# remi-or/fa2_triton

Hardware: AMD Instinct MI355X
Metric: attention TFLOP/s (fwd & fwd+bwd) at S=4096 D=128 bf16; % of MFMA peak (higher is better)
Workload: dtype bf16; 1 GPU; B=8 Hq=32 Hkv=32 S=4096 D=128 bf16 causal fwd+bwd per GPU (BASELINE.json configs[2]; configs[3] = B=64 batch-sharded over 8 GPUs); config=cfg3, global_batch=8, per_gpu_batch=8, seq_len=4096, heads=32, heads_kv=32, head_dim=128, causal=True, fwd_only=False, bias=False

## Files before the change

### fa2_triton_amd/csrc/dkdv_hp_kernel.h

```cpp
#pragma once
#include "common.h"
#include "fa2_internal.h"
#include "hp_unit.h"

namespace fa2 {

struct DkdvHpArgs {
  uint32_t qb0, qb1, vb0, vb1, ta, tb, lb, qoff0, qoff1, ooff0, ooff1, lsoff;
  uint32_t qb0h, qb1h, tah, tbh;
  int lr;
  int ng, nmt, c0, c01, c012, mlast, lq, kd0;
  uint32_t qrb, orb, qwrap, owrap, lwrap, lc0;
  uint32_t qlo, qhi, olo, ohi, lselo, lsehi, dllo, dlhi, mlds, lbs, w0;
  float sc;
  uint32_t mlo, mhi, mrange, mstep, mwrap;
  uint32_t dscb;
};

}

#include "gen/dkdv_hp_body.h"

namespace fa2 {

template <bool BF16, bool CAUSAL, bool DROPOUT>
FA2_DEV void dkdv_hp_main(const u32x4 (&kf)[16], const DkdvHpArgs& a) {
  if constexpr (DROPOUT) {
    if constexpr (BF16 && CAUSAL) dkdv_hp_main_bf16_causal_drop(kf, a);
    else if constexpr (BF16) dkdv_hp_main_bf16_full_drop(kf, a);
    else if constexpr (CAUSAL) dkdv_hp_main_f16_causal_drop(kf, a);
    else dkdv_hp_main_f16_full_drop(kf, a);
  } else {
    if constexpr (BF16 && CAUSAL) dkdv_hp_main_bf16_causal(kf, a);
    else if constexpr (BF16) dkdv_hp_main_bf16_full(kf, a);
    else if constexpr (CAUSAL) dkdv_hp_main_f16_causal(kf, a);
    else dkdv_hp_main_f16_full(kf, a);
  }
}

static_assert(DkdvLds<false>::v0 == 16384 * DkdvLds<false>::nbuf && DkdvLds<true>::rows == DkdvLds<true>::v0 + 65536,
              "dK/dV LDS layout");
constexpr int kDkdvStage = 32768;

struct DkdvBlk {
  int b, hkv, split, h0, G, Lq, Lk, n0, diag, n_mt, m_last, total;
};

template <bool CAUSAL>
FA2_DEV DkdvBlk dkdv_blk(const fa2_bwd_args& p, int nsplit, int item, int rep) {
  constexpr int BNK = 256, BMQ = 32;
  const int nkb = hp_blocks(p.seqlen_k), per_grp = hp_items_per_group<CAUSAL>(nkb);
  const int grp = item / per_grp, jb = item - grp * per_grp;
  DkdvBlk k;
  const int bkv = grp / nsplit;
  k.split = grp - bkv * nsplit;
  k.b = bkv / p.heads_kv;
  k.hkv = bkv - k.b * p.heads_kv;
  k.G = p.heads_q / p.heads_kv / nsplit;
  k.h0 = (k.hkv * nsplit + k.split) * k.G;
  k.Lq = p.seqlen_q;
  k.Lk = p.seqlen_k;
  if (p.cu_seqlens) k.Lq = k.Lk = p.cu_seqlens[k.b + 1] - p.cu_seqlens[k.b];
  k.n0 = (rep == 0 ? jb : nkb - 1 - jb) * BNK;
  k.diag = k.Lk - k.Lq;
  int m_begin = 0;
  if (CAUSAL) m_begin = max(0, k.n0 - k.diag) & ~(BMQ - 1);
  k.n_mt = (k.n0 < k.Lk && m_begin < k.Lq) ? (k.Lq - m_begin + BMQ - 1) / BMQ : 0;
  k.m_last = m_begin + (k.n_mt - 1) * BMQ;
  k.total = k.n_mt * k.G;
  return k;
}

FA2_DEV int dkdv_tiles_from(const DkdvBlk& k, int t) {
  return k.m_last < t ? 0 : min(((k.m_last - t) >> 5) + 1, k.n_mt);
}

template <bool CAUSAL>
FA2_DEV void dkdv_sched_dims(const fa2_bwd_args& p, int nsplit, int& T, int& nkb, int& per_grp) {
  nkb = hp_blocks(p.seqlen_k);
  per_grp = hp_items_per_group<CAUSAL>(nkb);
  T = per_grp * p.batch * p.heads_kv * nsplit;
}

FA2_DEV int64_t dkdv_mask_bytes(const fa2_bwd_args& p) {
  return 128ll * p.batch * p.heads_q * ((p.seqlen_q + 31) >> 5) * ((p.seqlen_k + 31) >> 5);
}
FA2_DEV uint32_t dkdv_mask_range(const fa2_bwd_args& p, int64_t off) {
  const int64_t r = dkdv_mask_bytes(p) - off;
  return r <= 0 ? 0u : r >= 0xFFFFFFFFll ? 0xFFFFFFFFu : (uint32_t)r;
}
FA2_DEV int64_t dkdv_mask_base(const fa2_bwd_args& p, const DkdvBlk& k, int w) {
  const int nrb = (p.seqlen_q + 31) >> 5, ncw = (p.seqlen_k + 31) >> 5;
  const int rt_min = (k.m_last >> 5) - (k.n_mt - 1);
  const int kt0 = (k.n0 + 64 * w) >> 5;
  return 128ll * (((int64_t)(k.b * p.heads_q + k.h0) * nrb + rt_min) * ncw + kt0);
}

typedef const __attribute__((address_space(4))) fa2_bwd_args* dkdv_kargs_t;
FA2_DEV const fa2_bwd_args* dkdv_kargs() {
  dkdv_kargs_t pa = (dkdv_kargs_t)__builtin_amdgcn_kernarg_segment_ptr();
  asm volatile("" : "+s"(pa));
  return (const fa2_bwd_args*)pa;
}

FA2_DEV int dkdv_lane() {
  int lane;
  asm volatile("v_mbcnt_lo_u32_b32 %0, -1, 0\n\tv_mbcnt_hi_u32_b32 %0, -1, %0" : "=v"(lane));
  return lane;
}

template <bool CAUSAL, bool DROPOUT>
FA2_DEV uint32_t dkdv_hp_issue(const fa2_bwd_args& p, const DkdvBlk& k, char* smem, int w, int lane, u32x4 (&kf)[16],
                               bool live = true) {
  constexpr int DT = 128, BMQ = 32, NT = 256;
  const int tid = 64 * w + lane, r32 = lane & 31, hh = lane >> 5, D = p.head_dim;
  const int kw0 = k.n0 + 64 * w;
  const uint32_t sb = lds_addr(smem);
  uint32_t tok = 0;
  if (live && k.total > 0) {
    const uint16_t* vg = (const uint16_t*)p.v + k.b * p.v_stride[0] + k.hkv * p.v_stride[2];
    BufStager<DT, 64, 64> vst;
    vst.init(lane, p.v_stride[1], D);
    tok = vst.issue(smem + DkdvLds<DROPOUT>::v0 + 16384 * w, vg, p.v_stride[1], kw0, k.Lk, BufStager<DT, 64, 64>::max_rows(p.v_stride[1]));
    BufStager<DT, BMQ, NT> qst, ost;
    qst.init(tid, p.q_stride[1], D);
    ost.init(tid, p.do_stride[1], D);
    const uint16_t* q0 = (const uint16_t*)p.q + k.b * p.q_stride[0] + k.h0 * p.q_stride[2];
    const uint16_t* o0 = (const uint16_t*)p.dout + k.b * p.do_stride[0] + k.h0 * p.do_stride[2];
    tok += qst.issue(smem, q0, p.q_stride[1], k.m_last, k.Lq, BufStager<DT, BMQ, NT>::max_rows(p.q_stride[1]));
    tok += ost.issue(smem + 8192, o0, p.do_stride[1], k.m_last, k.Lq, BufStager<DT, BMQ, NT>::max_rows(p.do_stride[1]));
    const int64_t l0 = (int64_t)(k.b * p.heads_q + k.h0) * p.lse_row_stride + k.m_last;
    if (w == 0) {
      const uint32_t nb = (uint32_t)min(k.Lq - k.m_last, BMQ) * 4u;
      blds4_lo32(4u * (uint32_t)lane, make_rsrc(p.lse + l0, nb), __builtin_amdgcn_readfirstlane(sb + DkdvLds<DROPOUT>::rows));
      blds4_lo32(4u * (uint32_t)lane, make_rsrc(p.delta + l0, nb), __builtin_amdgcn_readfirstlane(sb + DkdvLds<DROPOUT>::rows + 128));
    }
    if constexpr (DROPOUT) {
      const int ncw = (p.seqlen_k + 31) >> 5;
      const int64_t moff = dkdv_mask_base(p, k, w) + 128ll * ncw * (k.n_mt - 1);
      const char* mw = (const char*)p.dropout_mask + moff;
      blds4(4u * (uint32_t)lane, make_rsrc(mw, min(dkdv_mask_range(p, moff), 256u)), __builtin_amdgcn_readfirstlane(sb + DkdvLds<DROPOUT>::words + 256 * w));
    }
  }
#pragma unroll
  for (int kb = 0; kb < 2; ++kb) {
    const int kj = kw0 + 32 * kb + r32;
    const bool kval = kj < k.Lk;
    const uint16_t* krow = (const uint16_t*)p.k + k.b * p.k_stride[0] + k.hkv * p.k_stride[2] + (int64_t)(kval ? kj : 0) * p.k_stride[1];
#pragma unroll
    for (int ks = 0; ks < 8; ++ks) kf[kb * 8 + ks] = load_row_frag<true>(krow, 16 * ks + 8 * hh, D, kval);
  }
  return __builtin_amdgcn_readfirstlane(tok);
}

template <bool BF16, bool CAUSAL, bool DROPOUT>
__global__ void __launch_bounds__(256, 1) dkdv_hp_kernel(const fa2_bwd_args p_, int nsplit
#if FA2_HP_STAMPS
                                                         , unsigned long long* stamps
#endif
) {
  HpStamps st;
  constexpr int DT = 128, BMQ = 32, NT = 256;
  __shared__ __attribute__((aligned(16))) char smem[DkdvLds<DROPOUT>::size];

  const int w_ = __builtin_amdgcn_readfirstlane(threadIdx.x >> 6);
  int w = w_;
  PersistSched sch;
  {
    int T, nkb, per_grp;
    dkdv_sched_dims<CAUSAL>(p_, nsplit, T, nkb, per_grp);
    if (!sch.first(T, nkb, per_grp, CAUSAL)) return;
  }
  u32x4 kf[16];
  {
    const int lane = dkdv_lane();
    const auto& p = *dkdv_kargs();
    (void)dkdv_hp_issue<CAUSAL, DROPOUT>(p, dkdv_blk<CAUSAL>(p, nsplit, sch.item, sch.rep), smem, w, lane, kf);
  }

  st.start();
  while (true) {
    const int lane = dkdv_lane();
    w = w_;
    asm volatile("" : "+s"(w));
    const int tid = 64 * w + lane, r32 = lane & 31, hh = lane >> 5;
    {
      const auto& p = *dkdv_kargs();
      const DkdvBlk k = dkdv_blk<CAUSAL>(p, nsplit, sch.item, sch.rep);
      const int D = p.head_dim;
      const int kw0 = k.n0 + 64 * w;
      const float sc = p.softmax_scale * kLog2e;
      const uint32_t sb = lds_addr(smem);
      BufStager<DT, BMQ, NT> qst, ost;
      qst.init(tid, p.q_stride[1], D);
      ost.init(tid, p.do_stride[1], D);
      const int64_t q_rb = p.q_stride[1] * 2, o_rb = p.do_stride[1] * 2;
      const uint16_t* q0 = (const uint16_t*)p.q + k.b * p.q_stride[0] + k.h0 * p.q_stride[2];
      const uint16_t* o0 = (const uint16_t*)p.dout + k.b * p.do_stride[0] + k.h0 * p.do_stride[2];
      const int64_t l0 = (int64_t)(k.b * p.heads_q + k.h0) * p.lse_row_stride + k.m_last;

      DkdvHpArgs a;
      a.qb0 = hp_row_frag_base(sb, r32, hh, 0);
      a.qb1 = hp_row_frag_base(sb, r32, hh, 1);
      a.vb0 = a.qb0 + DkdvLds<DROPOUT>::v0 + 16384 * w;
      a.vb1 = a.qb1 + DkdvLds<DROPOUT>::v0 + 16384 * w;
      {
        const int i = lane & 15, g = lane >> 4, h = lane >> 5;
        const int qq = i >> 2, pq = i & 3;
        const int cc = 2 * (g & 1) + (pq >> 1);
        const int base = (4 * h + qq) * 64 + 8 * (pq & 1);
        a.ta = sb + base + ((cc ^ h) << 4);
        a.tb = sb + base + 512 + ((cc ^ h ^ 2) << 4);
      }
      a.qb0h = a.qb0 + 65536;
      a.qb1h = a.qb1 + 65536;
      a.tah = a.ta + 65536;
      a.tbh = a.tb + 65536;
      a.lb = sb + DkdvLds<DROPOUT>::rows + 16 * hh;
      a.qoff0 = qst.voff[0];
      a.qoff1 = qst.voff[1];
      a.ooff0 = ost.voff[0];
      a.ooff1 = ost.voff[1];
      a.lsoff = 4 * lane;
      a.lr = r32 - 4 * hh;
      a.kd0 = __builtin_amdgcn_readfirstlane(kw0 - k.diag);
      int c0, c1, c2;
      {
        const int live = kw0 >= k.Lk ? 0 : CAUSAL ? dkdv_tiles_from(k, kw0 - (BMQ - 1) - k.diag) : k.n_mt;
        const int clear = kw0 + 63 >= k.Lk ? 0 : CAUSAL ? dkdv_tiles_from(k, kw0 + 63 - k.diag) : k.n_mt;
        const int tail = k.m_last + BMQ > k.Lq ? 1 : 0;
        c1 = max(min(clear, live) - tail, 0);
        c0 = c1 > 0 ? tail : live;
        c2 = c1 > 0 ? live - clear : 0;
      }
      a.ng = __builtin_amdgcn_readfirstlane(k.G);
      a.nmt = __builtin_amdgcn_readfirstlane(k.n_mt);
      a.c0 = __builtin_amdgcn_readfirstlane(c0);
      a.c01 = __builtin_amdgcn_readfirstlane(c0 + c1);
      a.c012 = __builtin_amdgcn_readfirstlane(c0 + c1 + c2);
      a.mlast = __builtin_amdgcn_readfirstlane(k.m_last);
      a.lq = __builtin_amdgcn_readfirstlane(k.Lq);
      a.qrb = __builtin_amdgcn_readfirstlane((uint32_t)q_rb);
      a.orb = __builtin_amdgcn_readfirstlane((uint32_t)o_rb);
      a.qwrap = __builtin_amdgcn_readfirstlane((uint32_t)((int64_t)(k.n_mt - 1) * BMQ * q_rb + 2 * p.q_stride[2]));
      a.owrap = __builtin_amdgcn_readfirstlane((uint32_t)((int64_t)(k.n_mt - 1) * BMQ * o_rb + 2 * p.do_stride[2]));
      a.lwrap = __builtin_amdgcn_readfirstlane((uint32_t)(((int64_t)(k.n_mt - 1) * BMQ + p.lse_row_stride) * 4));
      a.lc0 = __builtin_amdgcn_readfirstlane((uint32_t)(l0 * 4));
      const uint64_t qa = (uint64_t)(uintptr_t)q0 + (uint64_t)((int64_t)k.m_last * q_rb);
      const uint64_t oa = (uint64_t)(uintptr_t)o0 + (uint64_t)((int64_t)k.m_last * o_rb);
      a.qlo = sgpr_lo(qa), a.qhi = sgpr_hi(qa);
      a.olo = sgpr_lo(oa), a.ohi = sgpr_hi(oa);
      const uint64_t la = (uint64_t)(uintptr_t)p.lse, da = (uint64_t)(uintptr_t)p.delta;
      a.lselo = sgpr_lo(la), a.lsehi = sgpr_hi(la);
      a.dllo = sgpr_lo(da), a.dlhi = sgpr_hi(da);
      a.mlds = __builtin_amdgcn_readfirstlane(sb + (uint32_t)w * 1024u);
      a.lbs = __builtin_amdgcn_readfirstlane(sb + (uint32_t)DkdvLds<DROPOUT>::rows);
      a.w0 = __builtin_amdgcn_readfirstlane((uint32_t)w);
      a.sc = sc;
      if constexpr (DROPOUT) {
        const uint32_t lds_part = sb + (uint32_t)DkdvLds<DROPOUT>::words + 256u * (uint32_t)w;
        a.lsoff = lds_part + 4 * lane;
        const int nrb = (p.seqlen_q + 31) >> 5, ncw = (p.seqlen_k + 31) >> 5;
        const uint64_t mb = ((uint64_t)(uintptr_t)p.dropout_mask + (uint64_t)dkdv_mask_base(p, k, w) - lds_part) & kAddr48;
        a.mlo = sgpr_lo(mb), a.mhi = sgpr_hi(mb);
        a.mrange = __builtin_amdgcn_readfirstlane(dkdv_mask_range(p, dkdv_mask_base(p, k, w) - (int64_t)lds_part));
        a.mstep = __builtin_amdgcn_readfirstlane((uint32_t)(128 * ncw));
        a.mwrap = __builtin_amdgcn_readfirstlane((uint32_t)(128 * ncw * (nrb + k.n_mt - 1)));
        a.dscb = __float_as_uint(1.f / (1.f - p.dropout_p));
        const uint64_t la2 = la - lds_part, da2 = da - lds_part;
        a.lselo = sgpr_lo(la2), a.lsehi = sgpr_hi(la2);
        a.dllo = sgpr_lo(da2), a.dlhi = sgpr_hi(da2);
      }

      st.mark(7);
      dkdv_hp_main<BF16, CAUSAL, DROPOUT>(kf, a);
      st.mark(0);
      st.count(5);
    }

    PersistSched nsch = sch;
    bool has_next;
    {
      const auto& p = *dkdv_kargs();
      int T, nkb, per_grp;
      dkdv_sched_dims<CAUSAL>(p, nsplit, T, nkb, per_grp);
      has_next = nsch.next(T, nkb, per_grp, CAUSAL);
    }
    uint32_t tok;
    {
      const auto& p = *dkdv_kargs();
      tok = dkdv_hp_issue<CAUSAL, DROPOUT>(p, dkdv_blk<CAUSAL>(p, nsplit, has_next ? nsch.item : sch.item, has_next ? nsch.rep : sch.rep), smem,
                                  w, lane, kf, has_next);
    }
    asm volatile("" ::: "memory");
    st.mark(1);

    {
      const auto& p = *dkdv_kargs();
      const DkdvBlk k = dkdv_blk<CAUSAL>(p, nsplit, sch.item, sch.rep);
      const int D = p.head_dim;
      const int kw0 = k.n0 + 64 * w;
      const float scale = p.softmax_scale;
      const float vscale = DROPOUT ? 1.f / (1.f - p.dropout_p) : 1.f;
#pragma unroll
      for (int kb = 0; kb < 2; ++kb) {
        f32x16 dv[4], dk[4];
        if (kb == 0) dkdv_hp_read<0>(dv, dk, tok);
        else dkdv_hp_read<1>(dv, dk, tok);
        st.mark(kb ? 4 : 2);
        const int kwb = kw0 + 32 * kb;
        const int kj = kwb + r32;
        const bool kval = kj < k.Lk;
        if (nsplit > 1) {
          if (kj < p.seqlen_k) {
            const int64_t row = (((int64_t)k.split * p.batch + k.b) * p.heads_kv + k.hkv) * p.seqlen_k + kj;
            float* pk = p.dkv_workspace + row * D;
            float* pv = p.dkv_workspace + ((int64_t)nsplit * p.batch * p.heads_kv * p.seqlen_k + row) * D;
#pragma unroll
            for (int dt = 0; dt < 4; ++dt)
#pragma unroll
              for (int g4 = 0; g4 < 4; ++g4) {
                const int d0 = 32 * dt + 8 * g4 + 4 * hh;
                f32x4 x, y;
#pragma unroll
                for (int j = 0; j < 4; ++j) {
                  x[j] = kval ? dk[dt][4 * g4 + j] : 0.f;
                  y[j] = kval ? dv[dt][4 * g4 + j] * vscale : 0.f;
                }
                *(f32x4*)(pk + d0) = x;
                *(f32x4*)(pv + d0) = y;
              }
          }
        } else if (kwb < p.seqlen_k) {
          uint16_t* k0 = (uint16_t*)p.dk + k.b * p.dk_stride[0] + k.hkv * p.dk_stride[2] + (int64_t)kwb * p.dk_stride[1];
          uint16_t* v0 = (uint16_t*)p.dv + k.b * p.dv_stride[0] + k.hkv * p.dv_stride[2] + (int64_t)kwb * p.dv_stride[1];
          const int nrows = min(32, p.seqlen_k - kwb);
          char* stage = smem + kDkdvStage + w * 32 * DT * 2;
          store_rows_lds<BF16, DT>(stage, dk, scale, kval, k0, p.dk_stride[1], nrows, D, lane, st.parts());
          store_rows_lds<BF16, DT>(stage, dv, vscale, kval, v0, p.dv_stride[1], nrows, D, lane, st.parts());
        }
        st.mark(kb ? 6 : 3);
      }
    }
    if (!has_next) break;
    sch = nsch;
  }
  asm volatile("s_waitcnt vmcnt(0)" ::: "memory");
#if FA2_HP_STAMPS
  st.flush(stamps, dkdv_lane());
#endif
}

template <bool BF16, bool CAUSAL, bool DROPOUT>
static void launch_dkdv_hp(const fa2_bwd_args& a, int nsplit, LaunchCtx ctx) {
  const int64_t items = hp_sched_items<CAUSAL>(a.seqlen_k, (int64_t)a.batch * a.heads_kv * nsplit);
  dim3 grid((unsigned)hp_grid(items, device_cu_count(), ctx.policy));
#if FA2_HP_STAMPS
  hipLaunchKernelGGL((dkdv_hp_kernel<BF16, CAUSAL, DROPOUT>), grid, dim3(256), 0, ctx.stream, a, nsplit, hp_stamp_buf());
#else
  hipLaunchKernelGGL((dkdv_hp_kernel<BF16, CAUSAL, DROPOUT>), grid, dim3(256), 0, ctx.stream, a, nsplit);
#endif
}

}
```

### fa2_triton_amd/csrc/dq_hp_kernel.h

```cpp
#pragma once
#include "common.h"
#include "fa2_internal.h"
#include "hp_unit.h"

namespace fa2 {

struct DqHpArgs {
  uint32_t kb0, kb1, ta, tb;
  uint32_t off0, off1, off2, off3;
  int rel0, rel1;
  float lse0, lse1, del0, del1;
  int na, last, ntiles;
  uint32_t tileb, kbytes, mlds, klo, khi, vlo, vhi;
  float sc;
  int boff;
  uint32_t nklo, nkhi, nvlo, nvhi, nkbytes, nqlo, nqhi, nqbytes, nolo, nohi, nobytes;
  uint32_t nqo0, noo0;
  uint32_t nqrs, nors;
  u32x4 mdesc;
  uint32_t mo0, nmo0, msh, mrs;
  float dsc;
};

}

#include "gen/dq_hp_body.h"

namespace fa2 {

template <bool BF16, bool CAUSAL, bool DROPOUT>
FA2_DEV void dq_hp_main(u32x4 (&q)[16], u32x4 (&o)[16], const DqHpArgs& a, uint32_t (&mw)[4]) {
  if constexpr (DROPOUT) {
    if constexpr (BF16 && CAUSAL) dq_hp_main_bf16_causal_drop(q, o, a, mw);
    else if constexpr (BF16) dq_hp_main_bf16_full_drop(q, o, a, mw);
    else if constexpr (CAUSAL) dq_hp_main_f16_causal_drop(q, o, a, mw);
    else dq_hp_main_f16_full_drop(q, o, a, mw);
  } else {
    if constexpr (BF16 && CAUSAL) dq_hp_main_bf16_causal(q, o, a);
    else if constexpr (BF16) dq_hp_main_bf16_full(q, o, a);
    else if constexpr (CAUSAL) dq_hp_main_f16_causal(q, o, a);
    else dq_hp_main_f16_full(q, o, a);
  }
}

template <bool CAUSAL>
struct DqHpUnit : HpRowUnit<CAUSAL> {
  const uint16_t *kg, *vg, *qg, *dg, *og;
  FA2_DEV void init(const fa2_bwd_args& p, HpWalk at) {
    const int hkv = HpRowUnit<CAUSAL>::init(p.heads_q, p.heads_kv, p.seqlen_q, p.seqlen_k, p.cu_seqlens, at.bh, at.mb);
    const int b = this->b, hq = this->hq;
    kg = (const uint16_t*)p.k + b * p.k_stride[0] + hkv * p.k_stride[2];
    vg = (const uint16_t*)p.v + b * p.v_stride[0] + hkv * p.v_stride[2];
    qg = (const uint16_t*)p.q + b * p.q_stride[0] + hq * p.q_stride[2];
    dg = (const uint16_t*)p.dout + b * p.do_stride[0] + hq * p.do_stride[2];
    og = (const uint16_t*)p.o + b * p.o_stride[0] + hq * p.o_stride[2];
  }
};

template <bool BF16, bool CAUSAL>
FA2_DEV void dq_hp_unit_rows(const fa2_bwd_args& p, const DqHpUnit<CAUSAL>& u, int qw0, int hh, int r32,
                             const u32x4 (&of)[16], float (&lse)[2], float (&del)[2]) {
  using E = Elem<BF16>;
  const int D = p.head_dim;
  const int64_t srow = (int64_t)(u.b * p.heads_q + u.hq) * p.lse_row_stride;
#pragma unroll
  for (int rb = 0; rb < 2; ++rb) {
    const int qi = qw0 + 32 * rb + r32;
    const bool qvalid = qi < u.Lq;
    const uint16_t* orow = u.og + (int64_t)(qvalid ? qi : 0) * p.o_stride[1];
    float part = 0.f;
#pragma unroll
    for (int ks = 0; ks < 8; ++ks) {
      const u32x4 orr = load_row_frag<true>(orow, 16 * ks + 8 * hh, D, qvalid);
      const u32x4 dr = of[rb * 8 + ks];
#pragma unroll
      for (int j = 0; j < 4; ++j) {
        part = fmaf(E::to_f32((uint16_t)(orr[j] & 0xFFFF)), E::to_f32((uint16_t)(dr[j] & 0xFFFF)), part);
        part = fmaf(E::to_f32((uint16_t)(orr[j] >> 16)), E::to_f32((uint16_t)(dr[j] >> 16)), part);
      }
    }
    del[rb] = qvalid ? half_sum(part) : 0.f;
    if (hh == 0 && qi < p.lse_row_stride) p.delta[srow + qi] = -del[rb];
    lse[rb] = qvalid ? p.lse[srow + qi] : 0.f;
  }
}

template <bool BF16, bool CAUSAL, bool DROPOUT>
__global__ void __launch_bounds__(256, 1) dq_hp_kernel(const fa2_bwd_args p
#if FA2_HP_STAMPS
                                                       , unsigned long long* stamps
#endif
) {
  HpStamps st;
  constexpr int DT = 128, BN = 64, NT = 256;
  constexpr int TILE = BN * DT * 2;
  __shared__ __attribute__((aligned(16))) char smem[4 * TILE + 4 * 32 * DT * 2];

  const int w = __builtin_amdgcn_readfirstlane(threadIdx.x >> 6);
  constexpr bool PAIR = CAUSAL;
  const int nmb = hp_blocks(p.seqlen_q), per_bh = hp_items_per_group<PAIR>(nmb);
  const int T = per_bh * p.batch * p.heads_q;
  PersistSched sch;
  if (!sch.first(T, nmb, per_bh, PAIR)) return;

  int tid = threadIdx.x;
  const int lane = tid & 63, r32 = lane & 31, hh = lane >> 5;
  const int D = p.head_dim;
  const float scale = p.softmax_scale, sc = scale * kLog2e;
  const uint32_t sb = lds_addr(smem);
  const uint32_t rowb = (uint32_t)(p.k_stride[1] * 2);
  const uint32_t qrowb = (uint32_t)(p.q_stride[1] * 2), orowb = (uint32_t)(p.do_stride[1] * 2);
  BufStager<DT, BN, NT> kst;
  kst.init(tid, p.k_stride[1], D);
  const int mrows = BufStager<DT, BN, NT>::max_rows(p.k_stride[1]);

  DqHpUnit<CAUSAL> u;
  u.init(p, hp_walk_unit(sch, nmb, per_bh, PAIR));
  u32x4 qf[16], of[16];
  float lse[2], del[2];
  {
    if (u.ntiles > 0) {
      kst.issue(smem, u.kg, p.k_stride[1], 0, u.Lk, mrows);
      kst.issue(smem + 2 * TILE, u.vg, p.v_stride[1], 0, u.Lk, mrows);
    }
    const int qw0 = u.m0 + 64 * w;
#pragma unroll
    for (int rb = 0; rb < 2; ++rb) {
      const int qi = qw0 + 32 * rb + r32;
      const bool qvalid = qi < u.Lq;
      const uint16_t* qrow = u.qg + (int64_t)(qvalid ? qi : 0) * p.q_stride[1];
      const uint16_t* drow = u.dg + (int64_t)(qvalid ? qi : 0) * p.do_stride[1];
#pragma unroll
      for (int ks = 0; ks < 8; ++ks) {
        qf[rb * 8 + ks] = load_row_frag<true>(qrow, 16 * ks + 8 * hh, D, qvalid);
        of[rb * 8 + ks] = load_row_frag<true>(drow, 16 * ks + 8 * hh, D, qvalid);
      }
    }
    dq_hp_unit_rows<BF16, CAUSAL>(p, u, qw0, hh, r32, of, lse, del);
  }
  int boff = 0;
  const int nrb = (p.seqlen_q + 31) >> 5, ncw = (p.seqlen_k + 31) >> 5;
  const uint32_t mbytes = DROPOUT ? (uint32_t)((int64_t)p.batch * p.heads_q * nrb * ncw * 128) : 0u;
  auto mask_off = [&](const DqHpUnit<CAUSAL>& x, int rb) -> uint32_t {
    const int rbi = (x.m0 + 64 * w + 32 * rb) >> 5;
    return (uint32_t)(((int64_t)(x.b * p.heads_q + x.hq) * nrb + rbi) * ncw * 128) + 4u * r32;
  };
  uint32_t mw[4] = {0u, 0u, 0u, 0u};
  if constexpr (DROPOUT) {
#pragma unroll
    for (int rb = 0; rb < 2; ++rb)
#pragma unroll
      for (int h = 0; h < 2; ++h) {
        const uint32_t off = mask_off(u, rb) + 128u * h;
        mw[2 * rb + h] = off < mbytes ? p.dropout_mask[off >> 2] : 0u;
      }
  }

  st.start();
  while (true) {
    asm volatile("" : "+v"(tid));
    const int qw0 = u.m0 + 64 * w;
    const int diag = u.Lk - u.Lq;
    PersistSched nsch = sch;
    const bool has_next = nsch.next(T, nmb, per_bh, PAIR);
    DqHpUnit<CAUSAL> nu;
    nu.init(p, hp_walk_unit(has_next ? nsch : sch, nmb, per_bh, PAIR));
    auto next_rows = [&](DqHpArgs& x) {
      const int nqw0 = nu.m0 + 64 * w;
      const int nrows = has_next ? min(max(nu.Lq - nqw0, 0), 64) : 0;
      const int64_t r0 = nrows > 0 ? nqw0 : 0;
      const uint16_t *nq = nu.qg + r0 * p.q_stride[1], *no = nu.dg + r0 * p.do_stride[1];
      x.nqlo = sgpr_lo(nq), x.nqhi = sgpr_hi(nq);
      x.nolo = sgpr_lo(no), x.nohi = sgpr_hi(no);
      x.nqbytes = __builtin_amdgcn_readfirstlane(row_range_bytes(nrows, qrowb));
      x.nobytes = __builtin_amdgcn_readfirstlane(row_range_bytes(nrows, orowb));
      x.nqo0 = (uint32_t)r32 * qrowb + 16u * hh;
      x.noo0 = (uint32_t)r32 * orowb + 16u * hh;
      x.nqrs = __builtin_amdgcn_readfirstlane(32u * qrowb);
      x.nors = __builtin_amdgcn_readfirstlane(32u * orowb);
    };

    DqHpArgs a;
    a.kb0 = hp_row_frag_base(sb, r32, hh, 0);
    a.kb1 = hp_row_frag_base(sb, r32, hh, 1);
    {
      const int i = lane & 15, g = lane >> 4, h = lane >> 5;
      const int qq = i >> 2, pq = i & 3;
      const int cc = 2 * (g & 1) + (pq >> 1);
      const int base = (4 * h + qq) * 64 + 8 * (pq & 1);
      a.ta = sb + base + ((cc ^ h) << 4);
      a.tb = sb + base + 512 + ((cc ^ h ^ 2) << 4);
    }
    a.off0 = kst.voff[0];
    a.off1 = kst.voff[1];
    a.off2 = kst.voff[2];
    a.off3 = kst.voff[3];
#pragma unroll
    for (int rb = 0; rb < 2; ++rb) {
      const int qi = qw0 + 32 * rb + r32;
      const int lim = qi >= u.Lq ? 0 : (CAUSAL ? min(u.Lk, qi + diag + 1) : u.Lk);
      (rb ? a.rel1 : a.rel0) = lim - 4 * hh;
    }
    a.lse0 = lse[0];
    a.lse1 = lse[1];
    a.del0 = del[0];
    a.del1 = del[1];
    const int ntiles = u.ntiles;
    int n_full = u.Lk / BN;
    if (CAUSAL) n_full = min(n_full, qw0 + diag + 1 >= 0 ? (qw0 + diag + 1) / BN : 0);
    const bool live0 = ntiles > 0 && !(CAUSAL && 0 > qw0 + 63 + diag);
    int last = -1;
    if (live0) {
      last = ntiles - 1;
      if (CAUSAL) last = min(last, (qw0 + 63 + diag) / BN);
    }
    a.na = __builtin_amdgcn_readfirstlane(min(n_full, last + 1));
    a.last = __builtin_amdgcn_readfirstlane(last);
    a.ntiles = __builtin_amdgcn_readfirstlane(ntiles);
    a.tileb = __builtin_amdgcn_readfirstlane(BN * rowb);
    a.kbytes = __builtin_amdgcn_readfirstlane(kv_range_bytes(u.Lk, mrows, rowb));
    a.mlds = __builtin_amdgcn_readfirstlane(sb + (uint32_t)w * 1024u);
    a.klo = sgpr_lo(u.kg), a.khi = sgpr_hi(u.kg);
    a.vlo = sgpr_lo(u.vg), a.vhi = sgpr_hi(u.vg);
    a.sc = sc;
    a.boff = __builtin_amdgcn_readfirstlane(boff);
    {
      a.nklo = sgpr_lo(nu.kg), a.nkhi = sgpr_hi(nu.kg);
      a.nvlo = sgpr_lo(nu.vg), a.nvhi = sgpr_hi(nu.vg);
      a.nkbytes = __builtin_amdgcn_readfirstlane(has_next && nu.ntiles > 0 ? kv_range_bytes(nu.Lk, mrows, rowb) : 0u);
      if constexpr (!DROPOUT) next_rows(a);
    }
    if constexpr (DROPOUT) {
      a.mo0 = mask_off(u, 0);
      a.nmo0 = has_next ? mask_off(nu, 0) : 0x7FFFFFF0u;
      a.mrs = __builtin_amdgcn_readfirstlane((uint32_t)ncw * 128u);
      a.msh = 4u * hh;
      const uint64_t ma = (uint64_t)(uintptr_t)p.dropout_mask & kAddr48;
      a.mdesc[0] = sgpr_lo(ma), a.mdesc[1] = sgpr_hi(ma);
      a.mdesc[2] = __builtin_amdgcn_readfirstlane(mbytes);
      a.mdesc[3] = 0x20000u;
      a.dsc = 1.f / (1.f - p.dropout_p);
    }

    st.mark(8);
    dq_hp_main<BF16, CAUSAL, DROPOUT>(qf, of, a, mw);
    st.mark(0);
    st.count(5);
    f32x16 acc[2][4];
    dq_hp_read(acc);
    st.mark(2);

    char* stage = smem + 4 * TILE + w * 32 * DT * 2;
#pragma unroll
    for (int rb = 0; rb < 2; ++rb) {
      const int r0 = qw0 + 32 * rb;
      if (r0 < p.seqlen_q) {
        const bool qvalid = r0 + r32 < u.Lq;
        uint16_t* q0 = (uint16_t*)p.dq + u.b * p.dq_stride[0] + u.hq * p.dq_stride[2] + (int64_t)r0 * p.dq_stride[1];
        store_rows_lds<BF16, DT>(stage, acc[rb], scale, qvalid, q0, p.dq_stride[1], min(32, p.seqlen_q - r0), D, lane, st.parts());
      }
      st.mark(3 + rb);
    }
    if (!has_next) break;
    if constexpr (DROPOUT) {
      DqHpArgs na;
      next_rows(na);
      dq_hp_load_next(qf, of, na);
      st.mark(12);
    }
    asm volatile("s_nop 14\n\ts_waitcnt vmcnt(0)"
                 : "+a"(qf[0]), "+a"(qf[1]), "+a"(qf[2]), "+a"(qf[3]), "+a"(qf[4]), "+a"(qf[5]), "+a"(qf[6]),
                   "+a"(qf[7]), "+a"(qf[8]), "+a"(qf[9]), "+a"(qf[10]), "+a"(qf[11]), "+a"(qf[12]), "+a"(qf[13]),
                   "+a"(qf[14]), "+a"(qf[15]), "+a"(of[0]), "+a"(of[1]), "+a"(of[2]), "+a"(of[3]), "+a"(of[4]),
                   "+a"(of[5]), "+a"(of[6]), "+a"(of[7]), "+a"(of[8]), "+a"(of[9]), "+a"(of[10]), "+a"(of[11]),
                   "+a"(of[12]), "+a"(of[13]), "+a"(of[14]), "+a"(of[15]), "+v"(mw[0]), "+v"(mw[1]), "+v"(mw[2]),
                   "+v"(mw[3])
                 :
                 : "memory");
    st.mark(6);
    dq_hp_unit_rows<BF16, CAUSAL>(p, nu, nu.m0 + 64 * w, hh, r32, of, lse, del);
    st.mark(7);
    boff = (boff + ntiles) & 1;
    sch = nsch;
    u = nu;
  }
  asm volatile("s_waitcnt vmcnt(0)" ::: "memory");
#if FA2_HP_STAMPS
  st.flush(stamps, lane);
#endif
}

template <bool BF16, bool CAUSAL, bool DROPOUT>
static void launch_dq_hp(const fa2_bwd_args& a, LaunchCtx ctx) {
  const int64_t items = hp_sched_items<CAUSAL>(a.seqlen_q, (int64_t)a.batch * a.heads_q);
  dim3 grid((unsigned)hp_grid(items, device_cu_count(), ctx.policy));
#if FA2_HP_STAMPS
  hipLaunchKernelGGL((dq_hp_kernel<BF16, CAUSAL, DROPOUT>), grid, dim3(256), 0, ctx.stream, a, hp_stamp_buf());
#else
  hipLaunchKernelGGL((dq_hp_kernel<BF16, CAUSAL, DROPOUT>), grid, dim3(256), 0, ctx.stream, a);
#endif
}

}
```

### fa2_triton_amd/csrc/hp_unit.h

```cpp
#pragma once
#include <stdint.h>

#ifdef __HIP__
#define FA2_HD __host__ __device__ __forceinline__
#else
#define FA2_HD inline
#endif

namespace fa2 {
constexpr int kHpBlock = 256;
constexpr int kHpTile = 64;

FA2_HD int hp_min(int a, int b) { return a < b ? a : b; }
FA2_HD int hp_max(int a, int b) { return a > b ? a : b; }

template <bool CAUSAL>
struct HpRowUnit {
  int b, hq, Lq, Lk, m0, ntiles;
  FA2_HD int init(int heads_q, int heads_kv, int seqlen_q, int seqlen_k, const int32_t* cu_seqlens, int bh, int mb) {
    b = bh / heads_q;
    hq = bh - b * heads_q;
    const int hkv = hq / (heads_q / heads_kv);
    Lq = seqlen_q;
    Lk = seqlen_k;
    if (cu_seqlens) {
      const int cu = cu_seqlens[b];
      Lq = Lk = cu_seqlens[b + 1] - cu;
    }
    m0 = mb * kHpBlock;
    int n_end = 0;
    if (m0 < Lq) {
      n_end = Lk;
      if (CAUSAL) n_end = hp_min(Lk, m0 + kHpBlock + Lk - Lq);
      n_end = hp_max(n_end, 0);
    }
    ntiles = (n_end + kHpTile - 1) / kHpTile;
    return hkv;
  }
};

template <bool CAUSAL>
FA2_HD int hp_n_full(int Lk, int diag, int qw0) {
  int n_full = Lk / kHpTile;
  if (CAUSAL) n_full = hp_min(n_full, qw0 + diag + 1 >= 0 ? (qw0 + diag + 1) / kHpTile : 0);
  return n_full;
}
template <bool CAUSAL>
FA2_HD int hp_last_tile(int diag, int qw0, int ntiles) {
  const bool live0 = ntiles > 0 && !(CAUSAL && 0 > qw0 + 63 + diag);
  int last = -1;
  if (live0) {
    last = ntiles - 1;
    if (CAUSAL) last = hp_min(last, (qw0 + 63 + diag) / kHpTile);
  }
  return last;
}

FA2_HD int hp_blocks(int seqlen) { return (seqlen + kHpBlock - 1) / kHpBlock; }
template <bool PAIR>
FA2_HD int hp_items_per_group(int n) { return PAIR ? (n + 1) / 2 : n; }
template <bool PAIR>
FA2_HD int64_t hp_sched_items(int seqlen, int64_t groups) { return hp_items_per_group<PAIR>(hp_blocks(seqlen)) * groups; }

FA2_HD uint32_t kv_range_bytes(int Lk, int mrows, uint32_t rowb) { return (uint32_t)hp_min(Lk, mrows) * rowb; }
FA2_HD uint32_t row_range_bytes(int nrows, uint32_t rowb) { return nrows > 0 ? (uint32_t)(nrows - 1) * rowb + 256u : 0u; }
}

#ifdef __HIP__
#include "common.h"
namespace fa2 {
struct HpWalk { int bh, mb; };
FA2_DEV HpWalk hp_walk_unit(const PersistSched& s, int nmb, int per_bh, bool pair) {
  HpWalk r;
  r.bh = s.item / per_bh;
  const int mbi = s.item - r.bh * per_bh;
  r.mb = pair && s.rep == 0 ? nmb - 1 - mbi : mbi;
  return r;
}

FA2_DEV uint32_t sgpr_lo(uint64_t a) { return __builtin_amdgcn_readfirstlane((uint32_t)a); }
FA2_DEV uint32_t sgpr_hi(uint64_t a) { return __builtin_amdgcn_readfirstlane((uint32_t)(a >> 32)); }
FA2_DEV uint32_t sgpr_lo(const void* p) { return sgpr_lo((uint64_t)(uintptr_t)p); }
FA2_DEV uint32_t sgpr_hi(const void* p) { return sgpr_hi((uint64_t)(uintptr_t)p); }
constexpr uint64_t kAddr48 = 0xFFFFFFFFFFFFull;
}
#endif
```

### fa2_triton_amd/csrc/select.h

```cpp
#pragma once
#include <stdint.h>

#include "fa2_amd.h"

namespace fa2 {

inline bool path_enabled(const fa2_policy* policy, uint32_t bit) { return !(policy && (policy->disable & bit)); }
inline int hp_grid(int64_t items, int ncu, const fa2_policy* policy) {
  const int cap = policy ? policy->grid_cap : 0;
  if (cap > 0 && cap < ncu) ncu = cap;
  return (int)(items < ncu ? items : ncu);
}

inline int head_dim_tile(int d) { return d <= 32 ? 32 : d <= 64 ? 64 : d <= 128 ? 128 : d <= 256 ? 256 : 0; }

inline bool bias16_rows(const void* bias, int dtype, const int64_t* stride) {
  return bias && (dtype == 16 || dtype == 17) && ((uintptr_t)bias & 15) == 0 && stride[0] % 8 == 0 &&
         stride[1] % 8 == 0 && stride[2] % 8 == 0;
}

inline bool fwd_hp_ok(const fa2_fwd_args& a, bool aligned, const fa2_policy* policy) {
  if (!path_enabled(policy, FA2_PATH_FWD_HP) || !aligned || a.head_dim != 128 || a.bias) return false;
#if FA2_HP_STAMPS
  if (a.dropout_p > 0.f) return false;
#endif
  if (a.dropout_p > 0.f &&
      (!a.dropout_mask || (int64_t)a.batch * a.heads_q * ((a.seqlen_q + 31) / 32) * ((a.seqlen_k + 31) / 32) * 128 >= ((int64_t)1 << 31)))
    return false;
  if (a.k_stride[1] != a.v_stride[1]) return false;
  return (int64_t)(a.seqlen_k + 128) * a.k_stride[1] * 2 < ((int64_t)1 << 31);
}

inline bool dq_hp_ok(const fa2_bwd_args& a, bool aligned, const fa2_policy* policy) {
  if (!path_enabled(policy, FA2_PATH_DQ_HP) || !aligned || a.head_dim != 128 || a.bias || a.dq_dtype != a.dtype) return false;
  if (a.dropout_p > 0.f) {
    if (!a.dropout_mask) return false;
    const int64_t nrb = (a.seqlen_q + 31) / 32, ncw = (a.seqlen_k + 31) / 32;
    if ((int64_t)a.batch * a.heads_q * nrb * ncw * 128 >= ((int64_t)1 << 31)) return false;
  }
  if (a.k_stride[1] != a.v_stride[1]) return false;
  const int64_t lim = (int64_t)1 << 31;
  return (int64_t)(a.seqlen_k + 128) * a.k_stride[1] * 2 < lim && (int64_t)64 * a.q_stride[1] * 2 < lim &&
         (int64_t)64 * a.do_stride[1] * 2 < lim;
}

inline bool dkdv_hp_ok(const fa2_bwd_args& a, bool aligned, const fa2_policy* policy) {
  if (!path_enabled(policy, FA2_PATH_DKDV_HP) || !aligned || a.head_dim != 128 || a.bias) return false;
  const int64_t lim = (int64_t)1 << 31;
  if (a.dropout_p > 0.f) {
    if (!a.dropout_mask || a.q_stride[1] != a.do_stride[1]) return false;
    const int64_t nrb = (a.seqlen_q + 31) / 32, ncw = (a.seqlen_k + 31) / 32;
    if ((int64_t)(a.heads_q / a.heads_kv) * nrb * ncw * 128 >= lim) return false;
  }
  const int64_t lse_bytes = (int64_t)a.batch * a.heads_q * a.lse_row_stride * 4;
  if (a.q_stride[2] < 0 || a.do_stride[2] < 0) return false;
  return (int64_t)(a.seqlen_q + 64) * a.q_stride[1] * 2 + 2 * a.q_stride[2] < lim &&
         (int64_t)(a.seqlen_q + 64) * a.do_stride[1] * 2 + 2 * a.do_stride[2] < lim && lse_bytes < lim;
}

constexpr int kDkvTargetGrid = 512;
inline int dkv_split_count(int B, int Hq, int Hkv, int Sk) {
  if (B < 1 || Hkv < 1 || Hq % Hkv != 0 || Sk < 1) return 1;
  const int G = Hq / Hkv;
  const int64_t grid = (int64_t)((Sk + 127) / 128) * B * Hkv;
  if (G <= 1 || grid >= kDkvTargetGrid) return 1;
  for (int s = 2; s < G; ++s)
    if (G % s == 0 && grid * s >= kDkvTargetGrid) return s;
  return G;
}
inline int64_t dkv_workspace_bytes(int B, int Hq, int Hkv, int Sk, int D) {
  const int s = dkv_split_count(B, Hq, Hkv, Sk);
  return s > 1 ? 2 * (int64_t)s * B * Hkv * Sk * D * 4 : 0;
}
inline int dkv_split(const fa2_bwd_args& a) {
  return a.dkv_workspace ? dkv_split_count(a.batch, a.heads_q, a.heads_kv, a.seqlen_k) : 1;
}

enum class Path : int { general, pipelined, hand_placed, local };

struct FwdPlan {
  Path path;
  bool causal, aligned, mask_first;
  int biask, drop;
};

inline FwdPlan select_fwd(const fa2_fwd_args& a, bool aligned, const fa2_policy* policy) {
  const bool bias = a.bias != nullptr, dropout = a.dropout_p > 0.f;
  if (a.local) return {Path::local, false, aligned, false, 0, 0};
  const int drop = dropout ? (a.dropout_mask ? 2 : 1) : 0, dt = head_dim_tile(a.head_dim);
  FwdPlan p = {Path::general, a.causal != 0, aligned, drop == 2, bias ? 1 : 0, drop};
  if (fwd_hp_ok(a, aligned, policy)) {
    p.path = Path::hand_placed;
  } else if ((dt == 64 || dt == 128) && aligned && !dropout && a.k_stride[1] == a.v_stride[1] &&
             (!bias || bias16_rows(a.bias, a.bias_dtype, a.bias_stride))) {
    p.path = Path::pipelined;
    p.biask = !bias ? 0 : (a.bias_dtype == FA2_BF16 ? 17 : 16);
  }
  return p;
}

enum class Stage : int { delta, dq, dbias, dkdv };
struct BwdPlan {
  bool causal, dropout, aligned, dq_f32;
  int biask;
  struct {
    Stage kind;
    Path path;
  } stage[4];
  int nstages;
  int nsplit;
  bool reduce;
};

inline BwdPlan select_bwd(const fa2_bwd_args& a, bool aligned, int stages, const fa2_policy* policy) {
  BwdPlan p = {};
  const bool bias = a.bias != nullptr;
  p.causal = !a.local && a.causal != 0;
  p.dropout = a.dropout_p > 0.f;
  p.aligned = aligned;
  p.dq_f32 = a.dq_dtype == FA2_F32;
  p.nsplit = 1;
  if (bias) p.biask = aligned && bias16_rows(a.bias, a.bias_dtype, a.bias_stride) ? (a.bias_dtype == FA2_BF16 ? 17 : 16) : 1;
  const Path local_or = a.local ? Path::local : Path::general;
  auto add = [&](Stage kind, Path path) {
    p.stage[p.nstages].kind = kind;
    p.stage[p.nstages++].path = path;
  };
  if ((stages & 1) && a.lse_row_stride > 0) add(Stage::delta, Path::general);
  if ((stages & 4) && a.seqlen_q > 0) add(Stage::dq, !a.local && dq_hp_ok(a, aligned, policy) ? Path::hand_placed : local_or);
  if ((stages & 8) && bias && a.dbias && a.seqlen_q > 0 && a.seqlen_k > 0) add(Stage::dbias, Path::general);
  if ((stages & 2) && a.seqlen_k > 0) {
    add(Stage::dkdv, !a.local && dkdv_hp_ok(a, aligned, policy) ? Path::hand_placed : local_or);
    if (!a.local) p.nsplit = dkv_split(a);
    p.reduce = p.nsplit > 1;
  }
  return p;
}

inline const fa2_kvcache_args& kv_base(const fa2_kvcache_args& a) { return a; }
inline const fa2_kvcache_args& kv_base(const fa2_paged_kvcache_args& a) { return a.base; }
inline const fa2_kvcache_args& kv_base(const fa2_fp8_kvcache_args& a) { return a.paged.base; }

inline int kv_row_tiles(const fa2_kvcache_args& a) {
  return (int)(((int64_t)(a.heads_q / a.heads_kv) * a.seqlen_q + 31) / 32);
}
inline int64_t kv_units(const fa2_kvcache_args& a) { return (int64_t)a.batch * a.heads_kv * kv_row_tiles(a); }

inline int kv_span_tiles(const fa2_kvcache_args& a) {
  int64_t span = a.capacity;
  if (a.window_left >= 0) {
    const int64_t band = (int64_t)a.window_left + a.seqlen_q + 63;
    if (band < span) span = band;
  }
  const int64_t t = (span + 63) / 64;
  return (int)(t < 1 ? 1 : t);
}

inline int kv_auto_splits(const fa2_kvcache_args& a, int ncu) {
  const int64_t units = kv_units(a);
  int64_t want = (2 * (int64_t)ncu + units - 1) / units;
  const int64_t most = kv_span_tiles(a) / FA2_KVCACHE_MIN_SPLIT_TILES;
  if (want > most) want = most;
  if (want > FA2_KVCACHE_MAX_SPLITS) want = FA2_KVCACHE_MAX_SPLITS;
  return (int)(want < 1 ? 1 : want);
}

inline int64_t kv_workspace_bytes(const fa2_kvcache_args& a, int nsplit) {
  if (nsplit <= 1) return 0;
  return (int64_t)nsplit * a.batch * a.heads_q * a.seqlen_q * ((int64_t)a.head_dim + 1) * 4;
}

constexpr int kFp8MaxHeadDim = 128;
inline int fp8_head_dim_tile(int d) { return d <= 64 ? 64 : d <= kFp8MaxHeadDim ? 128 : 0; }
inline bool fp8_paged(const fa2_fp8_kvcache_args& a) { return a.paged.block_table != nullptr; }
inline bool fp8_rows16(const void* cache, const int64_t* stride) {
  return ((uintptr_t)cache & 15) == 0 && stride[0] % 16 == 0 && stride[1] % 16 == 0 && stride[2] % 16 == 0;
}

}
```

Before: 940.2 TFLOP/s.

## Load K and O rows coalesced via buffer loads and transpose through LDS

In the dK/dV and dQ backward kernels, the per-lane strided row-fragment global loads for K (and for O in dQ's delta computation) are replaced. The new path issues coalesced 16-byte buffer loads across 4-row groups, then scatters them into a swizzled LDS image and reads them back in MFMA fragment layout. In dQ, the O request for the next unit is issued early so its latency overlaps the dQ store phase. This adds LDS traffic and register pressure for the raw staging arrays, and the hand-placed path now requires extra stride-eligibility checks.

Result: no change. 944.5 TFLOP/s, median of 6 (+0.5%).

```diff
diff --git a/fa2_triton_amd/csrc/dkdv_hp_kernel.h b/fa2_triton_amd/csrc/dkdv_hp_kernel.h
--- a/fa2_triton_amd/csrc/dkdv_hp_kernel.h
+++ b/fa2_triton_amd/csrc/dkdv_hp_kernel.h
@@ -110,10 +110,10 @@
 }
 
 template <bool CAUSAL, bool DROPOUT>
-FA2_DEV uint32_t dkdv_hp_issue(const fa2_bwd_args& p, const DkdvBlk& k, char* smem, int w, int lane, u32x4 (&kf)[16],
+FA2_DEV uint32_t dkdv_hp_issue(const fa2_bwd_args& p, const DkdvBlk& k, char* smem, int w, int lane, u32x4 (&kraw)[16],
                                bool live = true) {
   constexpr int DT = 128, BMQ = 32, NT = 256;
-  const int tid = 64 * w + lane, r32 = lane & 31, hh = lane >> 5, D = p.head_dim;
+  const int tid = 64 * w + lane, D = p.head_dim;
   const int kw0 = k.n0 + 64 * w;
   const uint32_t sb = lds_addr(smem);
   uint32_t tok = 0;
@@ -142,15 +142,16 @@
       blds4(4u * (uint32_t)lane, make_rsrc(mw, min(dkdv_mask_range(p, moff), 256u)), __builtin_amdgcn_readfirstlane(sb + DkdvLds<DROPOUT>::words + 256 * w));
     }
   }
-#pragma unroll
-  for (int kb = 0; kb < 2; ++kb) {
-    const int kj = kw0 + 32 * kb + r32;
-    const bool kval = kj < k.Lk;
-    const uint16_t* krow = (const uint16_t*)p.k + k.b * p.k_stride[0] + k.hkv * p.k_stride[2] + (int64_t)(kval ? kj : 0) * p.k_stride[1];
-#pragma unroll
-    for (int ks = 0; ks < 8; ++ks) kf[kb * 8 + ks] = load_row_frag<true>(krow, 16 * ks + 8 * hh, D, kval);
+  {
+    const int nrows = live ? hp_min(hp_max(k.Lk - kw0, 0), 64) : 0;
+    const uint16_t* k0 = (const uint16_t*)p.k + k.b * p.k_stride[0] + k.hkv * p.k_stride[2] + (int64_t)(nrows > 0 ? kw0 : 0) * p.k_stride[1];
+    hp_rows_request(kraw, k0, (uint32_t)(p.k_stride[1] * 2), nrows, lane);
   }
   return __builtin_amdgcn_readfirstlane(tok);
+}
+
+FA2_DEV void dkdv_hp_k_frags(u32x4 (&kf)[16], const u32x4 (&kraw)[16], char* smem, int w, int lane) {
+  hp_rows_frags(kf, kraw, smem + kDkdvStage + w * 8192, lane);
 }
 
 template <bool BF16, bool CAUSAL, bool DROPOUT>
@@ -175,7 +176,9 @@
   {
     const int lane = dkdv_lane();
     const auto& p = *dkdv_kargs();
-    (void)dkdv_hp_issue<CAUSAL, DROPOUT>(p, dkdv_blk<CAUSAL>(p, nsplit, sch.item, sch.rep), smem, w, lane, kf);
+    u32x4 kraw[16];
+    (void)dkdv_hp_issue<CAUSAL, DROPOUT>(p, dkdv_blk<CAUSAL>(p, nsplit, sch.item, sch.rep), smem, w, lane, kraw);
+    dkdv_hp_k_frags(kf, kraw, smem, w, lane);
   }
 
   st.start();
@@ -287,10 +290,11 @@
       has_next = nsch.next(T, nkb, per_grp, CAUSAL);
     }
     uint32_t tok;
+    u32x4 kraw[16];
     {
       const auto& p = *dkdv_kargs();
       tok = dkdv_hp_issue<CAUSAL, DROPOUT>(p, dkdv_blk<CAUSAL>(p, nsplit, has_next ? nsch.item : sch.item, has_next ? nsch.rep : sch.rep), smem,
-                                  w, lane, kf, has_next);
+                                  w, lane, kraw, has_next);
     }
     asm volatile("" ::: "memory");
     st.mark(1);
@@ -343,6 +347,8 @@
       }
     }
     if (!has_next) break;
+    dkdv_hp_k_frags(kf, kraw, smem, w, lane);
+    st.mark(8);
     sch = nsch;
   }
   asm volatile("s_waitcnt vmcnt(0)" ::: "memory");
diff --git a/fa2_triton_amd/csrc/dq_hp_kernel.h b/fa2_triton_amd/csrc/dq_hp_kernel.h
--- a/fa2_triton_amd/csrc/dq_hp_kernel.h
+++ b/fa2_triton_amd/csrc/dq_hp_kernel.h
@@ -57,21 +57,25 @@
   }
 };
 
+template <bool CAUSAL>
+FA2_DEV void dq_hp_request_o(u32x4 (&oraw)[16], const fa2_bwd_args& p, const DqHpUnit<CAUSAL>& u, int qw0, bool live, int lane) {
+  const int nrows = live ? min(max(u.Lq - qw0, 0), 64) : 0;
+  hp_rows_request(oraw, u.og + (int64_t)(nrows > 0 ? qw0 : 0) * p.o_stride[1], (uint32_t)(p.o_stride[1] * 2), nrows, lane);
+}
+
 template <bool BF16, bool CAUSAL>
 FA2_DEV void dq_hp_unit_rows(const fa2_bwd_args& p, const DqHpUnit<CAUSAL>& u, int qw0, int hh, int r32,
-                             const u32x4 (&of)[16], float (&lse)[2], float (&del)[2]) {
+                             const u32x4 (&of)[16], const u32x4 (&orf)[16], float (&lse)[2], float (&del)[2]) {
   using E = Elem<BF16>;
-  const int D = p.head_dim;
   const int64_t srow = (int64_t)(u.b * p.heads_q + u.hq) * p.lse_row_stride;
 #pragma unroll
   for (int rb = 0; rb < 2; ++rb) {
     const int qi = qw0 + 32 * rb + r32;
     const bool qvalid = qi < u.Lq;
-    const uint16_t* orow = u.og + (int64_t)(qvalid ? qi : 0) * p.o_stride[1];
     float part = 0.f;
 #pragma unroll
     for (int ks = 0; ks < 8; ++ks) {
-      const u32x4 orr = load_row_frag<true>(orow, 16 * ks + 8 * hh, D, qvalid);
+      const u32x4 orr = orf[rb * 8 + ks];
       const u32x4 dr = of[rb * 8 + ks];
 #pragma unroll
       for (int j = 0; j < 4; ++j) {
@@ -136,7 +140,10 @@
         of[rb * 8 + ks] = load_row_frag<true>(drow, 16 * ks + 8 * hh, D, qvalid);
       }
     }
-    dq_hp_unit_rows<BF16, CAUSAL>(p, u, qw0, hh, r32, of, lse, del);
+    u32x4 oraw[16], orf[16];
+    dq_hp_request_o<CAUSAL>(oraw, p, u, qw0, true, lane);
+    hp_rows_frags(orf, oraw, smem + 4 * TILE + w * 32 * DT * 2, lane);
+    dq_hp_unit_rows<BF16, CAUSAL>(p, u, qw0, hh, r32, of, orf, lse, del);
   }
   int boff = 0;
   const int nrb = (p.seqlen_q + 31) >> 5, ncw = (p.seqlen_k + 31) >> 5;
@@ -249,6 +256,10 @@
     f32x16 acc[2][4];
     dq_hp_read(acc);
     st.mark(2);
+    u32x4 oraw[16];
+    asm volatile("" ::: "memory");
+    dq_hp_request_o<CAUSAL>(oraw, p, nu, nu.m0 + 64 * w, has_next, lane);
+    asm volatile("" ::: "memory");
 
     char* stage = smem + 4 * TILE + w * 32 * DT * 2;
 #pragma unroll
@@ -278,7 +289,9 @@
                  :
                  : "memory");
     st.mark(6);
-    dq_hp_unit_rows<BF16, CAUSAL>(p, nu, nu.m0 + 64 * w, hh, r32, of, lse, del);
+    u32x4 orf[16];
+    hp_rows_frags(orf, oraw, stage, lane);
+    dq_hp_unit_rows<BF16, CAUSAL>(p, nu, nu.m0 + 64 * w, hh, r32, of, orf, lse, del);
     st.mark(7);
     boff = (boff + ntiles) & 1;
     sch = nsch;
diff --git a/fa2_triton_amd/csrc/hp_unit.h b/fa2_triton_amd/csrc/hp_unit.h
--- a/fa2_triton_amd/csrc/hp_unit.h
+++ b/fa2_triton_amd/csrc/hp_unit.h
@@ -64,6 +64,21 @@
 
 FA2_HD uint32_t kv_range_bytes(int Lk, int mrows, uint32_t rowb) { return (uint32_t)hp_min(Lk, mrows) * rowb; }
 FA2_HD uint32_t row_range_bytes(int nrows, uint32_t rowb) { return nrows > 0 ? (uint32_t)(nrows - 1) * rowb + 256u : 0u; }
+
+constexpr int kRowReqRows = 4;
+FA2_HD int hp_rowreq_row(int lane, int j) { return kRowReqRows * j + ((lane >> 2) & 3); }
+FA2_HD int hp_rowreq_chunk(int lane) { return ((lane >> 4) << 2) | (lane & 3); }
+FA2_HD uint32_t hp_rowreq_off(int lane, int j, uint32_t rowb) {
+  return (uint32_t)hp_rowreq_row(lane, j) * rowb + 16u * (uint32_t)hp_rowreq_chunk(lane);
+}
+FA2_HD bool hp_rowreq_in_range(uint32_t off, uint32_t range) { return off <= range && range - off >= 16u; }
+template <int ROWS>
+FA2_HD int hp_image_off(int r, int c) { return (c >> 2) * (ROWS * 64) + r * 64 + (((c & 3) ^ ((r >> 2) & 3)) << 4); }
+template <int ROWS>
+FA2_HD int hp_frag_off(int row, int ks, int hh) {
+  const int cc = ((ks & 1) << 1) | hh;
+  return (ks >> 1) * (ROWS * 64) + row * 64 + ((cc ^ ((row >> 2) & 3)) << 4);
+}
 }
 
 #ifdef __HIP__
@@ -83,5 +98,26 @@
 FA2_DEV uint32_t sgpr_lo(const void* p) { return sgpr_lo((uint64_t)(uintptr_t)p); }
 FA2_DEV uint32_t sgpr_hi(const void* p) { return sgpr_hi((uint64_t)(uintptr_t)p); }
 constexpr uint64_t kAddr48 = 0xFFFFFFFFFFFFull;
+
+FA2_DEV void hp_rows_request(u32x4 (&raw)[16], const uint16_t* g, uint32_t rowb, int nrows, int lane) {
+  asm volatile("" : "+v"(lane));
+  const uint64_t base = ((uint64_t)sgpr_hi(g) << 32) | sgpr_lo(g);
+  const __amdgpu_buffer_rsrc_t rsrc = __builtin_amdgcn_make_buffer_rsrc(
+      (void*)(uintptr_t)base, 0, (int)__builtin_amdgcn_readfirstlane(row_range_bytes(hp_min(nrows, 64), rowb)), 0x00020000);
+#pragma unroll
+  for (int j = 0; j < 16; ++j)
+    raw[j] = __builtin_bit_cast(u32x4, __builtin_amdgcn_raw_buffer_load_b128(rsrc, (int)hp_rowreq_off(lane, j, rowb), 0, 0));
+}
+FA2_DEV void hp_rows_frags(u32x4 (&f)[16], const u32x4 (&raw)[16], char* image, int lane) {
+  asm volatile("" : "+v"(lane));
+  const int r32 = lane & 31, hh = lane >> 5;
+#pragma unroll
+  for (int rb = 0; rb < 2; ++rb) {
+#pragma unroll
+    for (int j = 0; j < 8; ++j) *(u32x4*)(image + hp_image_off<32>(hp_rowreq_row(lane, j), hp_rowreq_chunk(lane))) = raw[8 * rb + j];
+#pragma unroll
+    for (int ks = 0; ks < 8; ++ks) f[8 * rb + ks] = *(const u32x4*)(image + hp_frag_off<32>(r32, ks, hh));
+  }
+}
 }
 #endif
diff --git a/fa2_triton_amd/csrc/select.h b/fa2_triton_amd/csrc/select.h
--- a/fa2_triton_amd/csrc/select.h
+++ b/fa2_triton_amd/csrc/select.h
@@ -40,6 +40,7 @@
   }
   if (a.k_stride[1] != a.v_stride[1]) return false;
   const int64_t lim = (int64_t)1 << 31;
+  if (a.o_stride[1] < 128 || (int64_t)64 * a.o_stride[1] * 2 >= lim) return false;
   return (int64_t)(a.seqlen_k + 128) * a.k_stride[1] * 2 < lim && (int64_t)64 * a.q_stride[1] * 2 < lim &&
          (int64_t)64 * a.do_stride[1] * 2 < lim;
 }
@@ -54,6 +55,7 @@
   }
   const int64_t lse_bytes = (int64_t)a.batch * a.heads_q * a.lse_row_stride * 4;
   if (a.q_stride[2] < 0 || a.do_stride[2] < 0) return false;
+  if (a.k_stride[1] < 128 || (int64_t)64 * a.k_stride[1] * 2 >= lim) return false;
   return (int64_t)(a.seqlen_q + 64) * a.q_stride[1] * 2 + 2 * a.q_stride[2] < lim &&
          (int64_t)(a.seqlen_q + 64) * a.do_stride[1] * 2 + 2 * a.do_stride[2] < lim && lse_bytes < lim;
 }
```
